# FengDushuo/BBBP-Multi-Modal-Deep-Ensemble-Framework

Measured on AMD Instinct MI355X. Metric: molecules/sec fwd+bwd (3-branch ensemble, B=512), higher is better.
Workload: dtype f32; 1 GPU; MixedInputModel F=167 (MACCS) + 3x128x128 image, 6-layer encoder + 2-stage CNN + fusion + BN head; forward + MSE + backward + fused AdamW, train mode (dropout 0.1); global_batch=512, per_gpu_batch=512, parallelism=dp1, input=device-resident

## Files before the change

bbbp-multi-modal-deep-ensemble-framework_amd/_lib.py:

```python
from __future__ import annotations

import ctypes
import os
import re
from ctypes import (POINTER, Structure, c_char_p, c_double, c_float, c_int, c_long, c_size_t, c_uint8, c_uint64, c_void_p)

_HERE = os.path.dirname(os.path.abspath(__file__))
LIB_PATH = os.environ.get("BBBP_LIB", os.path.join(_HERE, "libbbbp_hip.so"))
HEADER_PATH = os.path.join(os.path.dirname(_HERE), "include", "bbbp_hip.h")

_lib = None


class MixedDesc(Structure):
    _fields_ = [("batch", c_int), ("fingerprint_size", c_int), ("nhead", c_int), ("num_layers", c_int),
                ("dim_feedforward", c_int), ("training", c_int), ("dropout_p", c_float), ("seed", c_uint64),
                ("need_input_grad", c_int), ("fusion", c_int), ("inference", c_int),
                ("world", c_int), ("rank", c_int), ("collective", c_void_p), ("collective_ctx", c_void_p)]


CollectiveFn = ctypes.CFUNCTYPE(c_int, c_void_p, c_int, c_int, c_int, ctypes.c_size_t, ctypes.c_size_t, ctypes.c_size_t, c_void_p)


class GemmDesc(Structure):
# ... 91 lines not shown
    "bbbp_mlp_profile": (c_int, [c_int, c_void_p]),
    "bbbp_mlp_profile_groups": (c_int, [c_void_p, c_int]),
    "bbbp_set_conv_wgrad_beside_encoder": (c_int, [c_int]),
    "bbbp_set_conv2_fwd_pipe": (c_int, [c_int]),
    "bbbp_adamw_step_deferred": (c_int, [c_void_p, c_void_p, c_void_p, c_void_p, c_void_p, c_long, c_long, c_long, c_double, c_double, c_double, c_double, c_double, c_int, c_double]),
    "bbbp_param_sync": (c_int, [c_void_p]),
    "bbbp_param_stream": (c_void_p, []),
    "bbbp_scale": (c_int, [c_void_p, _FP, c_long, c_float]),
    "bbbp_resize_bilinear_totensor": (c_int, [c_void_p, c_void_p, c_void_p, c_void_p, _FP, c_void_p, c_void_p, c_int, c_void_p,
                                              c_void_p, c_int, c_int, c_int, c_int, c_int, c_int]),
    "bbbp_standardize_chunk": (c_int, [c_void_p, c_void_p, _FP, _FP, _FP, c_void_p, c_void_p, c_int, c_int, c_int]),
    "bbbp_set_partition": (c_int, [c_int, c_size_t]),
    "bbbp_set_comm_cus": (c_int, [c_int]),
    "bbbp_set_ln_absorb": (c_int, [c_int]),
    "bbbp_set_overlap": (c_int, [c_int]),
    "bbbp_profile_enable": (c_int, [c_int]),
    "bbbp_profile_select": (c_int, [ctypes.c_uint]),
    "bbbp_profile_num_sections": (c_int, []),
    "bbbp_profile_section_name": (c_char_p, [c_int]),
    "bbbp_profile_collect": (c_int, [POINTER(c_float), POINTER(c_int)]),
    "bbbp_profile_timeline": (c_int, [POINTER(c_int), POINTER(c_float), POINTER(c_float), c_int]),
    "bbbp_mixed_num_params": (c_int, [POINTER(MixedDesc)]),
    "bbbp_mixed_workspace_bytes": (c_size_t, [POINTER(MixedDesc)]),
    "bbbp_mixed_forward": (c_int, [c_void_p, POINTER(MixedDesc), _PP, _PP, _FP, _FP, _FP, c_void_p, c_size_t]),
    "bbbp_mixed_backward": (c_int, [c_void_p, POINTER(MixedDesc), _PP, _PP, _FP, _FP, _FP, c_void_p, c_size_t]),
}


def declared_symbols():
    text = open(HEADER_PATH).read()
    text = re.sub(r"/\*.*?\*/", "", text, flags=re.S)
    return sorted(set(re.findall(r"\b(bbbp_[a-z0-9_]+)\s*\(", text)))


def lib() -> ctypes.CDLL:
    global _lib
    if _lib is not None:
        return _lib
    if not os.path.exists(LIB_PATH):
        raise RuntimeError(
            f"{LIB_PATH} is missing: build it with `python -c 'import __graft_entry__ as g; g.build()'` "
            "(hipcc --offload-arch=gfx950).  The BBBP hot path has no CPU fallback.")
    l = ctypes.CDLL(LIB_PATH)
    for name, (res, args) in _SIGNATURES.items():
        fn = getattr(l, name)
        fn.restype = res
# ... 15 lines not shown
```

bbbp-multi-modal-deep-ensemble-framework_amd/csrc/engine.hip:

```cpp
#include "common.h"
#include "attention_b3.h"
#include "encoder_sliced.h"
#include "head_sync.h"
#include <optional>
#include "bbbp_hip.h"
#include <mutex>
#include <stdlib.h>

namespace {

constexpr int IMG = 128, C1 = 32, C2 = 64, FC = 128, NHEADS_FUSION = 4, FUS_HID = 128;
constexpr int H1 = 256, H2 = 128, H3 = 64;
constexpr int COMB = 2 * FC;
constexpr int IMG_FLAT = C2 * (IMG / 4) * (IMG / 4);

enum { L_INW = 0, L_INB, L_OUTW, L_OUTB, L_W1, L_B1, L_W2, L_B2, L_N1W, L_N1B, L_N2W, L_N2B, L_COUNT };
struct PIdx {
    int L, NF;
    PIdx(int layers, int fusion) : L(layers), NF(fusion == 0 ? 4 * NHEADS_FUSION : 0) {}
    explicit PIdx(const bbbp_mixed_desc* d) : PIdx(d->num_layers, d->fusion) {}
    int layer(int l, int k) const { return l * L_COUNT + k; }
    int base() const { return L * L_COUNT; }
    int fpfc_w() const { return base() + 0; }
    int fpfc_b() const { return base() + 1; }
// ... 110 lines not shown
        o.z1 = b.f(B * F); o.y1 = b.f(B * F); o.hff = b.f(B * DFF); o.z2 = b.f(B * F); o.y2 = b.f(B * F);
        o.mean1 = b.f(B); o.rstd1 = b.f(B); o.mean2 = b.f(B); o.rstd2 = b.f(B);
    }
    if (p->L > 0 && bbbp_enc_sliced_supported(p->B, p->F, p->NH, p->DFF, p->L)) {
        p->sl_sync = b.take(bbbp_enc_sliced_sync_bytes());
        p->sl_part = b.take(bbbp_enc_sliced_part_bytes(p->B, p->F));
        p->sl_kvpart = p->inference ? 0 : b.take(bbbp_enc_sliced_kvpart_bytes(p->B, p->F));
    } else {
        p->sl_sync = p->sl_part = p->sl_kvpart = 0;
    }
    for (int l = 0; l < p->L; ++l) {
        p->fwf[l] = p->fold ? b.f(bbbp_outproj_fold_floats(p->F, 0)) : 0; p->fbf[l] = p->fold ? b.f(bbbp_outproj_fold_floats(p->F, 1)) : 0;
        p->fwvt[l] = p->fold ? b.f(bbbp_outproj_fold_floats(p->F, 2)) : 0;
        p->ftdw[l] = (p->fold && !p->inference) ? b.f(bbbp_outproj_fold_floats(p->F, 3)) : 0;
        p->ftdb[l] = (p->fold && !p->inference) ? b.f(bbbp_outproj_fold_floats(p->F, 4)) : 0;
    }
    p->attn_part_bytes = p->attn_b3 ? bbbp_attn_b3_workspace_bytes(p->B, p->NH, p->D) : 0;
    p->attn_part = p->attn_part_bytes ? b.take(p->attn_part_bytes) : 0;
    p->pool1 = b.f(B * C1 * (IMG / 2) * (IMG / 2)); p->mask1 = p->inference ? 0 : b.take(B * C1 * (IMG / 2) * (IMG / 2));
    p->pool2 = b.f(B * IMG_FLAT); p->mask2 = p->inference ? 0 : b.take(B * IMG_FLAT);
    p->combined = b.f(B * COMB); p->hid = b.f(NHEADS_FUSION * B * FUS_HID); p->attn = b.f(B * NHEADS_FUSION);
    p->fused = p->concat ? p->combined : b.f(B * COMB); p->h = b.f(B * H1); p->hb = b.f(B * H1); p->bn_mean = b.f(H1); p->bn_rstd = b.f(H1);
    p->h2 = b.f(B * H2); p->h3 = b.f(B * H3);
    p->head_partial = b.f((size_t)p->world * ((B + 15) / 16) * 2 * H1);
    size_t cw = bbbp_conv3x3_workspace_bytes(p->B, 32, 64, 64, 64);
    size_t cw1 = bbbp_conv3x3_workspace_bytes(p->B, 3, 32, 128, 128);
    size_t sb = cw > cw1 ? cw : cw1;
    size_t gw = bbbp_gemm_workspace_bytes(p->B, FC, IMG_FLAT, 1);
    if (gw > sb) sb = gw;
    if (sb < ((size_t)32 << 20)) sb = (size_t)32 << 20;
    p->scratch_bytes = sb;
    p->scratch = b.take(sb);
    p->scratch2_bytes = (size_t)32 << 20;
    p->scratch2 = b.take(p->scratch2_bytes);
    if (p->inference) { p->total = b.off; return BBBP_OK; }
    for (int l = 0; l < p->L; ++l) {
        LayerGrad& g = p->lgrad[l];
        g.dyout = b.f(B * F); g.dz2 = b.f(B * F); g.dz2d = p->drop ? b.f(B * F) : g.dz2; g.dhff = b.f(B * DFF);
        g.dy1 = b.f(B * F); g.dz1 = b.f(B * F); g.dz1d = p->drop ? b.f(B * F) : g.dz1; g.dqkv = b.f(B * 3 * F);
    }
    p->scratch3_bytes = (size_t)32 << 20;
    p->scratch3 = b.take(p->scratch3_bytes);
    p->dA = b.f(B * F); p->dB = b.f(B * F); p->dqkv = b.f(B * 3 * F); p->dprob = p->flash ? 0 : b.f(NH * B * Bg); p->dctx = b.f(B * F);
    p->dkvg = p->exact ? b.f(Bg * 2 * F) : 0; p->dkvl = p->exact ? b.f(B * 2 * F) : 0;
    p->dhff = b.f(B * DFF); p->dpool2 = b.f(B * IMG_FLAT); p->dpool1 = b.f(B * C1 * (IMG / 2) * (IMG / 2));
    p->dcomb = b.f(B * COMB); p->dfused = b.f(B * COMB); p->dlogit = b.f(NHEADS_FUSION * B);
    p->dpre = b.f(NHEADS_FUSION * B * FUS_HID); p->dh = b.f(B * H1); p->dhb = b.f(B * H1); p->dh2 = b.f(B * H2);
// ... 304 lines not shown
        ms_sum[g_prof.sec[i]] += ms;
        count[g_prof.sec[i]] += 1;
    }
    g_prof.n = 0;
    return BBBP_OK;
}

extern "C" int bbbp_profile_timeline(int* section, float* start_ms, float* end_ms, int max_entries) {
    BBBP_CHECK_ARG(section && start_ms && end_ms && max_entries >= 0, "profile_timeline: bad arguments");
    const int n = g_prof.n < max_entries ? g_prof.n : max_entries;
    for (int i = 0; i < n; ++i) {
        section[i] = g_prof.sec[i];
        BBBP_CHECK_HIP(hipEventElapsedTime(&start_ms[i], g_prof.a[0], g_prof.a[i]));
        BBBP_CHECK_HIP(hipEventElapsedTime(&end_ms[i], g_prof.a[0], g_prof.b[i]));
    }
    return n;
}

extern "C" int bbbp_mixed_num_params(const bbbp_mixed_desc* d) {
    if (!d) return -1;
    if (d->num_layers < 0 || d->num_layers > 32 || (d->fusion != 0 && d->fusion != 1)) return -1;
    return PIdx(d).count();
}

extern "C" size_t bbbp_mixed_workspace_bytes(const bbbp_mixed_desc* d) {
    Plan p;
    if (make_plan(d, &p)) return 0;
    return p.total;
}

static int forward_enqueue(void* stream, const bbbp_mixed_desc* d, const float* const* P, float* const* bn_running,
                           const float* fingerprint, const float* image, float* out, void* workspace,
                           size_t workspace_bytes) {
    Plan plan;
    TRY(make_plan(d, &plan));
    SeedScope seed_scope(reinterpret_cast<const unsigned long long*>(static_cast<char*>(workspace) + plan.seed_slot));
    BBBP_CHECK_ARG(P && fingerprint && image && out && workspace && bn_running, "mixed_forward: null pointer");
    if (workspace_bytes < plan.total) {
        bbbp_set_error("mixed_forward: workspace %zu < %zu bytes", workspace_bytes, plan.total);
        return BBBP_ERR_WORKSPACE;
    }
    Ctx c{static_cast<hipStream_t>(stream), static_cast<char*>(workspace), &plan};
    const PIdx ix(d);
    if (bbbp_param_pending_elsewhere(P[ix.ifc_w()])) (void)bbbp_param_wait(c.st, nullptr);
    const int B = plan.B, F = plan.F, NH = plan.NH, D = plan.D, DFF = plan.DFF;
    const int Bk = (int)plan.Bg;
// ... 212 lines not shown
    if (!fused_rows && !sliced) {
        if (pend.z) {
            TRY(bbbp_layernorm_linear_fwd(ce.st, pend.z, F, pend.gamma, pend.beta, 1e-5f, P[ix.fpfc_w()], P[ix.fpfc_b()], comb, COMB, BBBP_ACT_RELU, 0.f, 0,
                                          pend.y, F, pend.mean, pend.rstd, B, FC, F));
            pend.z = nullptr;
        } else {
            TRY(linear_fwd(ce, x, F, P[ix.fpfc_w()], P[ix.fpfc_b()], comb, COMB, B, FC, F, BBBP_ACT_RELU));
        }
    }
    sec_enc.reset();

    if (ss) TRY(join_side(c.st, ss));
    part.reset();
    Section sec_head(c.st, SEC_HEAD_FWD);

    static const int fused_head = [] { const char* e = getenv("BBBP_FUSED_HEAD"); return e ? atoi(e) : 1; }();
    BBBP_CHECK_ARG(!plan.exact || (fused_head && NHEADS_FUSION == 4), "the exact-global-batch mode needs the fused head (BBBP_FUSED_HEAD=1)");
    if (fused_head && NHEADS_FUSION == 4) {
        const float *fw1[4] = {}, *fb1[4] = {}, *fw2[4] = {}, *fb2[4] = {};
        if (!plan.concat)
            for (int h = 0; h < 4; ++h) { fw1[h] = P[ix.fus(h, 0)]; fb1[h] = P[ix.fus(h, 1)]; fw2[h] = P[ix.fus(h, 2)]; fb2[h] = P[ix.fus(h, 3)]; }
        bbbp_head_sync sync;
        sync.world = plan.world; sync.rank = plan.rank;
        const size_t pcount = (size_t)((B + 15) / 16) * 2 * H1;
        if (plan.exact)
            sync.between = [&]() -> int {
                return run_collective(d, BBBP_COLL_ALLGATHER, BBBP_COLL_BN_FWD, -1, plan.head_partial + (size_t)plan.rank * pcount * sizeof(float),
                                      plan.head_partial, pcount, c.st);
            };
        return bbbp_head_forward_fused_sync(c.st, comb, fw1, fb1, fw2, fb2, P[ix.fc0_w()], P[ix.fc0_b()], P[ix.bn_w()], P[ix.bn_b()],
                                            bn_running[0], bn_running[1], P[ix.fc3_w()], P[ix.fc3_b()], P[ix.fc5_w()], P[ix.fc5_b()],
                                            P[ix.fc7_w()], P[ix.fc7_b()], c.f(plan.hid), c.f(plan.attn), c.f(plan.fused), c.f(plan.h),
                                            c.f(plan.hb), c.f(plan.bn_mean), c.f(plan.bn_rstd), c.f(plan.h2), c.f(plan.h3), out,
                                            c.f(plan.head_partial), B, d->training, plan.concat ? 1 : 0, plan.exact ? &sync : nullptr);
    }
    float* hid = c.f(plan.hid);
    float* fused = c.f(plan.fused);
    if (!plan.concat) {
        const float* w2[NHEADS_FUSION]; const float* b2[NHEADS_FUSION];
        for (int h = 0; h < NHEADS_FUSION; ++h) {
            TRY(linear_fwd(c, comb, COMB, P[ix.fus(h, 0)], P[ix.fus(h, 1)], hid + (size_t)h * B * FUS_HID, FUS_HID, B, FUS_HID, COMB,
                           BBBP_ACT_TANH));
            w2[h] = P[ix.fus(h, 2)]; b2[h] = P[ix.fus(h, 3)];
        }
        TRY(bbbp_fusion_combine_fwd(c.st, comb, hid, w2, b2, fused, c.f(plan.attn), B, COMB, FUS_HID, NHEADS_FUSION));
    }

// ... 63 lines not shown
    float* dlogit = c.f(plan.dlogit); float* dpre = c.f(plan.dpre);
    bool head_leaves_pending = false;
    auto head_leaves = [&]() -> int {
        TRY(linear_bwd_weight_bias(cl, dout, 1, h3, H3, G[ix.fc7_w()], G[ix.fc7_b()], B, 1, H3));
        TRY(linear_bwd_weight_bias(cl, dh3, H3, h2, H2, G[ix.fc5_w()], G[ix.fc5_b()], B, H3, H2));
        TRY(linear_bwd_weight_bias(cl, dh2, H2, hb, H1, G[ix.fc3_w()], G[ix.fc3_b()], B, H2, H1));
        TRY(linear_bwd_weight_bias(cl, dh, H1, fused, COMB, G[ix.fc0_w()], G[ix.fc0_b()], B, H1, COMB));
        for (int hh = 0; hh < (plan.concat ? 0 : NHEADS_FUSION); ++hh) {
            float* dl = dlogit + (size_t)hh * B;
            float* dp = dpre + (size_t)hh * B * FUS_HID;
            const float* hd = hid + (size_t)hh * B * FUS_HID;
            TRY(linear_bwd_weight_bias(cl, dl, 1, hd, FUS_HID, G[ix.fus(hh, 2)], G[ix.fus(hh, 3)], B, 1, FUS_HID));
            TRY(linear_bwd_weight_bias(cl, dp, FUS_HID, comb, COMB, G[ix.fus(hh, 0)], G[ix.fus(hh, 1)], B, FUS_HID, COMB));
        }
        TRY(bbbp_bias_act_bwd(cl.st, dcomb + FC, COMB, nullptr, 0, G[ix.ifc_b()], B, FC, 0, 1.f));
        return BBBP_OK;
    };
    BBBP_CHECK_ARG(!plan.exact || fused_head_bwd, "the exact-global-batch mode needs the fused head backward (bbbp_set_fused_head_bwd(1))");
    if (fused_head_bwd) {
        const float* fw1[NHEADS_FUSION]; const float* fw2[NHEADS_FUSION];
        for (int hh = 0; hh < NHEADS_FUSION; ++hh) { fw1[hh] = P[ix.fus(hh, 0)]; fw2[hh] = P[ix.fus(hh, 2)]; }
        bbbp_head_sync sync;
        sync.world = plan.world; sync.rank = plan.rank;
        const size_t pcount = (size_t)((B + 15) / 16) * 2 * H1;
        if (plan.exact)
            sync.between = [&]() -> int {
                return run_collective(d, BBBP_COLL_ALLGATHER, BBBP_COLL_BN_BWD, -1, plan.head_partial + (size_t)plan.rank * pcount * sizeof(float),
                                      plan.head_partial, pcount, c.st);
            };
        TRY(bbbp_head_backward_fused_sync(c.st, dout, comb, hid, c.f(plan.attn), h, h2, h3, c.f(plan.bn_mean), c.f(plan.bn_rstd),
                                          P[ix.bn_w()], fw1, fw2, P[ix.fc0_w()], P[ix.fc3_w()], P[ix.fc5_w()], P[ix.fc7_w()], dh3, dh2, dhb,
                                          dh, dlogit, dpre, dcomb, G[ix.bn_w()], G[ix.bn_b()], c.f(plan.head_partial), B, d->training,
                                          plan.exact ? &sync : nullptr));
        TRY(leaf_after(c));
        head_leaves_pending = true;
    } else {
    TRY(linear_bwd_weight_bias(cl, dout, 1, h3, H3, G[ix.fc7_w()], G[ix.fc7_b()], B, 1, H3));
    {
        bbbp_gemm_desc g = gemm_desc(0, 0, B, H3, 1, 1.f, dout, 1, P[ix.fc7_w()], H3, dh3, H3);
        g.gate = h3; g.ldg = H3;
        TRY(bbbp_gemm_f32_grouped(c.st, &g, 1, c.scratch(), c.scratch_bytes()));
    }
    TRY(leaf_after(c));
    TRY(linear_bwd_weight_bias(cl, dh3, H3, h2, H2, G[ix.fc5_w()], G[ix.fc5_b()], B, H3, H2));
    {
        bbbp_gemm_desc g = gemm_desc(0, 0, B, H2, H3, 1.f, dh3, H3, P[ix.fc5_w()], H2, dh2, H2);
        g.gate = h2; g.ldg = H2;
// ... 470 lines not shown
```

bbbp-multi-modal-deep-ensemble-framework_amd/csrc/head.hip:

```cpp
#include "common.h"
#include "bbbp_hip.h"
#include "head_sync.h"

namespace {

constexpr int ROWS = 16;
constexpr int NTH = 512;
constexpr int NW = NTH / 64;
constexpr int COMB = 256, FHID = 128, NHEADS = 4, H1 = 256, H2 = 128, H3 = 64;
constexpr int LD = COMB + 4;
typedef float f32x4g __attribute__((ext_vector_type(4), aligned(4)));
static_assert(NTH >= H1, "one thread per BatchNorm column");

struct HeadParams {
    const float* comb;
    const float* fw1[NHEADS]; const float* fb1[NHEADS]; const float* fw2[NHEADS]; const float* fb2[NHEADS];
    const float* w0; const float* b0;
    const float* gamma; const float* beta; float* running_mean; float* running_var;
    const float* w3; const float* b3;
    const float* w5; const float* b5;
    const float* w7; const float* b7;
    float* hid; float* attn; float* fused; float* h; float* hb; float* bn_mean; float* bn_rstd; float* h2; float* h3; float* out;
    float* partial;
    int B, training;
    float eps, momentum;
    int concat;
    int world, rank;
};

template <int NCH>
__device__ __forceinline__ void load_b(f32x4 (&bf)[NCH], const float* Wrow ) {
#pragma unroll
    for (int c = 0; c < NCH; ++c) { f32x4g v = *reinterpret_cast<const f32x4g*>(Wrow + 16 * c); bf[c] = f32x4{v[0], v[1], v[2], v[3]}; }
}
template <int NCH>
__device__ __forceinline__ f32x4 mma_tile(const f32x4 (&af)[NCH], const f32x4 (&bf)[NCH]) {
    f32x4 acc0 = {0.f, 0.f, 0.f, 0.f}, acc1 = {0.f, 0.f, 0.f, 0.f};
#pragma unroll
    for (int c = 0; c < NCH; ++c)
#pragma unroll
        for (int j = 0; j < 4; j += 2) {
            acc0 = __builtin_amdgcn_mfma_f32_16x16x4f32(af[c][j], bf[c][j], acc0, 0, 0, 0);
            acc1 = __builtin_amdgcn_mfma_f32_16x16x4f32(af[c][j + 1], bf[c][j + 1], acc1, 0, 0, 0);
        }
    return acc0 + acc1;
}

template <int NCH>
__device__ __forceinline__ void load_a(f32x4 (&af)[NCH], const float* s, int ld, int lane) {
    const int i = lane & 15, kq = lane >> 4;
#pragma unroll
    for (int c = 0; c < NCH; ++c) af[c] = *reinterpret_cast<const f32x4*>(s + i * ld + 16 * c + 4 * kq);
}

__device__ __forceinline__ float sum16(float v) {
    v += __shfl_xor(v, 1); v += __shfl_xor(v, 2); v += __shfl_xor(v, 4); v += __shfl_xor(v, 8);
    return v;
}

__global__ __launch_bounds__(NTH) void head_a_kernel(HeadParams p) {
    __shared__ __attribute__((aligned(16))) float sC[ROWS * LD];
    __shared__ float sLogit[NW][NHEADS][ROWS];
    __shared__ float sP[ROWS][NHEADS];
    const int t = threadIdx.x, lane = t & 63, wave = t >> 6;
    const int q = lane & 15, kq = lane >> 4;
    const int r0 = blockIdx.x * ROWS, nrows = min(ROWS, p.B - r0);
    for (int idx = t; idx < ROWS * (COMB / 4); idx += NTH) {
        const int r = idx / (COMB / 4), c4 = idx % (COMB / 4);
        f32x4 v = {0.f, 0.f, 0.f, 0.f};
        if (r < nrows) v = *reinterpret_cast<const f32x4*>(p.comb + (long)(r0 + r) * COMB + c4 * 4);
        *reinterpret_cast<f32x4*>(sC + r * LD + c4 * 4) = v;
    }
    __syncthreads();
    f32x4 af[COMB / 16];
    load_a<COMB / 16>(af, sC, LD, lane);
    float lg[NHEADS][4];
    f32x4 bf[2][COMB / 16];
    const int n = wave * 16 + q;
    if (p.concat) {
        load_b<COMB / 16>(bf[0], p.w0 + (long)n * COMB + 4 * kq);
    } else {
    load_b<COMB / 16>(bf[0], p.fw1[0] + (long)n * COMB + 4 * kq);
#pragma unroll
    for (int h = 0; h < NHEADS; ++h) {
        if (h + 1 < NHEADS) load_b<COMB / 16>(bf[(h + 1) & 1], p.fw1[h + 1] + (long)n * COMB + 4 * kq);
        else load_b<COMB / 16>(bf[(h + 1) & 1], p.w0 + (long)n * COMB + 4 * kq);
        f32x4 acc = mma_tile<COMB / 16>(af, bf[h & 1]);
        const float b = p.fb1[h][n], w2 = p.fw2[h][n];
#pragma unroll
        for (int r = 0; r < 4; ++r) {
            const int row = 4 * kq + r;
            const float v = tanhf(acc[r] + b);
            if (row < nrows) p.hid[((long)h * p.B + r0 + row) * FHID + n] = v;
            lg[h][r] = sum16(v * w2);
        }
    }
    if (q == 0) {
#pragma unroll
        for (int h = 0; h < NHEADS; ++h)
#pragma unroll
            for (int r = 0; r < 4; ++r) sLogit[wave][h][4 * kq + r] = lg[h][r];
    }
    __syncthreads();
    if (t < ROWS) {
        float a[NHEADS], m = -INFINITY;
#pragma unroll
        for (int h = 0; h < NHEADS; ++h) {
            float z = 0.f;
#pragma unroll
            for (int w = 0; w < NW; ++w) z += sLogit[w][h][t];
            a[h] = z + p.fb2[h][0];
            m = fmaxf(m, a[h]);
        }
        float den = 0.f;
#pragma unroll
        for (int h = 0; h < NHEADS; ++h) { a[h] = __expf(a[h] - m); den += a[h]; }
#pragma unroll
        for (int h = 0; h < NHEADS; ++h) {
            a[h] /= den;
            sP[t][h] = a[h];
            if (t < nrows) p.attn[(long)(r0 + t) * NHEADS + h] = a[h];
        }
    }
    __syncthreads();
    for (int idx = t; idx < ROWS * COMB; idx += NTH) {
        const int r = idx / COMB, c = idx % COMB;
        const float x = sC[r * LD + c];
        float s = 0.f;
#pragma unroll
        for (int h = 0; h < NHEADS; ++h) s += sP[r][h] * x;
        sC[r * LD + c] = s;
        if (r < nrows) p.fused[(long)(r0 + r) * COMB + c] = s;
    }
    __syncthreads();
    load_a<COMB / 16>(af, sC, LD, lane);
    }
#pragma unroll
    for (int tt = 0; tt < 2; ++tt) {
        const int n0 = (wave + NW * tt) * 16 + q;
        if (tt == 0) load_b<COMB / 16>(bf[1], p.w0 + (long)((wave + NW) * 16 + q) * COMB + 4 * kq);
        f32x4 acc = mma_tile<COMB / 16>(af, bf[tt & 1]);
        const float b = p.b0[n0];
        float v[4], s = 0.f;
#pragma unroll
        for (int r = 0; r < 4; ++r) {
            const int row = 4 * kq + r;
            v[r] = fmaxf(acc[r] + b, 0.f);
            if (row < nrows) { p.h[(long)(r0 + row) * H1 + n0] = v[r]; s += v[r]; }
        }
        s += __shfl_xor(s, 16); s += __shfl_xor(s, 32);
        const float mean = s / nrows;
        float m2 = 0.f;
#pragma unroll
        for (int r = 0; r < 4; ++r) if (4 * kq + r < nrows) { const float d = v[r] - mean; m2 += d * d; }
        m2 += __shfl_xor(m2, 16); m2 += __shfl_xor(m2, 32);
        if (kq == 0) {
            const long slot = (long)p.rank * gridDim.x + blockIdx.x;
            p.partial[(slot * 2 + 0) * H1 + n0] = mean;
            p.partial[(slot * 2 + 1) * H1 + n0] = m2;
        }
    }
}

__global__ __launch_bounds__(NTH) void head_b_kernel(HeadParams p) {
    __shared__ __attribute__((aligned(16))) float sA[ROWS * LD];
    __shared__ __attribute__((aligned(16))) float sB[ROWS * (H2 + 4)];
    __shared__ __attribute__((aligned(16))) float sD[ROWS * (H3 + 4)];
    __shared__ float sMean[H1], sRstd[H1];
    const int t = threadIdx.x, lane = t & 63, wave = t >> 6;
    const int q = lane & 15, kq = lane >> 4;
    const int r0 = blockIdx.x * ROWS, nrows = min(ROWS, p.B - r0);
    const int nblocks = (p.B + ROWS - 1) / ROWS;
    f32x4 bf3[H1 / 16];
    load_b<H1 / 16>(bf3, p.w3 + (long)(wave * 16 + q) * H1 + 4 * kq);
    if (t < H1) {
        const int c = t;
        float mean, rstd;
        if (p.training) {
            float na = 0.f, ma = 0.f, m2a = 0.f;
            for (int b = 0; b < nblocks * p.world; ++b) {
                const float nb = (float)min(ROWS, p.B - (b % nblocks) * ROWS);
                const float mb = p.partial[((long)b * 2 + 0) * H1 + c], m2b = p.partial[((long)b * 2 + 1) * H1 + c];
                const float d = mb - ma, n = na + nb;
                ma += d * (nb / n);
                m2a += m2b + d * d * (na * nb / n);
                na = n;
            }
            const float nall = (float)p.B * (float)p.world;
            const float var = m2a / nall;
            mean = ma; rstd = rsqrtf(var + p.eps);
            if (blockIdx.x == 0) {
                p.running_mean[c] = (1.f - p.momentum) * p.running_mean[c] + p.momentum * mean;
                p.running_var[c] = (1.f - p.momentum) * p.running_var[c] + p.momentum * var * (nall / (nall - 1.f));
            }
        } else {
// ... 141 lines not shown
                    p.dhb[(long)(r0 + row) * H1 + n] = g;
                    pa += g * (p.h[(long)(r0 + row) * H1 + n] - mu) * rs;
                    pb += g;
                }
            }
            sPa[kq][n] = pa; sPb[kq][n] = pb;
        }
    }
    __syncthreads();
    if (t < H1) {
        const long slot = (long)p.rank * gridDim.x + blockIdx.x;
        p.partial[(slot * 2 + 0) * H1 + t] = ((sPa[0][t] + sPa[1][t]) + sPa[2][t]) + sPa[3][t];
        p.partial[(slot * 2 + 1) * H1 + t] = ((sPb[0][t] + sPb[1][t]) + sPb[2][t]) + sPb[3][t];
    }
}

__global__ __launch_bounds__(NTH) void head_bwd_c_kernel(HeadBwdParams p) {
    __shared__ __attribute__((aligned(16))) float sX[ROWS * LD];
    __shared__ __attribute__((aligned(16))) float sP[NHEADS * ROWS * LDP];
    __shared__ float sSa[H1], sSb[H1];
    const int t = threadIdx.x, lane = t & 63, wave = t >> 6;
    const int q = lane & 15, kq = lane >> 4;
    const int r0 = blockIdx.x * ROWS, nrows = min(ROWS, p.B - r0);
    const int nblocks = (p.B + ROWS - 1) / ROWS;
    if (t < H1) {
        float sa = 0.f, sb = 0.f, la = 0.f, lb = 0.f;
        for (int b = 0; b < nblocks * p.world; ++b) {
            const float va = p.partial[((long)b * 2 + 0) * H1 + t], vb = p.partial[((long)b * 2 + 1) * H1 + t];
            sa += va; sb += vb;
            if (b / nblocks == p.rank) { la += va; lb += vb; }
        }
        sSa[t] = sa; sSb[t] = sb;
        if (blockIdx.x == 0) { p.dgamma[t] = la; p.dbeta[t] = lb; }
    }
    __syncthreads();
    for (int idx = t; idx < ROWS * H1; idx += NTH) {
        const int r = idx / H1, c = idx % H1;
        float v = 0.f;
        if (r < nrows) {
            const float d = p.dhb[(long)(r0 + r) * H1 + c], xv = p.h[(long)(r0 + r) * H1 + c];
            const float g = p.gamma[c], mu = p.bn_mean[c], rs = p.bn_rstd[c];
            const float nall = (float)p.B * (float)p.world;
            v = p.training ? g * rs * (d - sSb[c] / nall - (xv - mu) * rs * (sSa[c] / nall)) : d * g * rs;
            v = xv > 0.f ? v : 0.f;
            p.dh[(long)(r0 + r) * H1 + c] = v;
        }
        sX[r * LD + c] = v;
// ... 38 lines not shown
                sP[(hh * ROWS + r) * LDP + c] = v;
            }
        }
    }
    __syncthreads();
    f32x4 acc[2] = {{0.f, 0.f, 0.f, 0.f}, {0.f, 0.f, 0.f, 0.f}};
#pragma unroll
    for (int hh = 0; hh < NHEADS; ++hh) mma_kmajor<FHID, 2>(acc, sP + hh * ROWS * LDP, LDP, p.fw1[hh], COMB, wave * 32, lane);
#pragma unroll
    for (int u = 0; u < 2; ++u) {
        const int n = wave * 32 + 2 * q + u;
#pragma unroll
        for (int r = 0; r < 4; ++r) {
            const int row = 4 * kq + r;
            if (row < nrows) {
                const float v = acc[u][r] + sX[row * LD + n];
                p.dcomb[(long)(r0 + row) * COMB + n] = p.comb[(long)(r0 + row) * COMB + n] > 0.f ? v : 0.f;
            }
        }
    }
}

}

int bbbp_head_forward_fused(hipStream_t st, const float* comb, const float* const* fw1, const float* const* fb1,
                            const float* const* fw2, const float* const* fb2, const float* w0, const float* b0, const float* gamma,
                            const float* beta, float* running_mean, float* running_var, const float* w3, const float* b3,
                            const float* w5, const float* b5, const float* w7, const float* b7, float* hid, float* attn, float* fused,
                            float* h, float* hb, float* bn_mean, float* bn_rstd, float* h2, float* h3, float* out, float* partial,
                            int B, int training, int concat) {
    return bbbp_head_forward_fused_sync(st, comb, fw1, fb1, fw2, fb2, w0, b0, gamma, beta, running_mean, running_var, w3, b3, w5, b5, w7, b7,
                                        hid, attn, fused, h, hb, bn_mean, bn_rstd, h2, h3, out, partial, B, training, concat, nullptr);
}

int bbbp_head_forward_fused_sync(hipStream_t st, const float* comb, const float* const* fw1, const float* const* fb1,
                                 const float* const* fw2, const float* const* fb2, const float* w0, const float* b0, const float* gamma,
                                 const float* beta, float* running_mean, float* running_var, const float* w3, const float* b3,
                                 const float* w5, const float* b5, const float* w7, const float* b7, float* hid, float* attn, float* fused,
                                 float* h, float* hb, float* bn_mean, float* bn_rstd, float* h2, float* h3, float* out, float* partial,
                                 int B, int training, int concat, const bbbp_head_sync* sync) {
    const int world = sync ? sync->world : 1, rank = sync ? sync->rank : 0;
    BBBP_CHECK_ARG(B >= 1, "head: empty batch");
    BBBP_CHECK_ARG(world >= 1 && rank >= 0 && rank < world, "head: rank %d of %d", rank, world);
    BBBP_CHECK_ARG(!(training && (long)B * world <= 1), "Expected more than 1 value per channel when training, got input size [%d, %d]", B, H1);
    HeadParams p;
    p.comb = comb;
    for (int i = 0; i < NHEADS; ++i) { p.fw1[i] = fw1[i]; p.fb1[i] = fb1[i]; p.fw2[i] = fw2[i]; p.fb2[i] = fb2[i]; }
    p.w0 = w0; p.b0 = b0; p.gamma = gamma; p.beta = beta; p.running_mean = running_mean; p.running_var = running_var;
    p.w3 = w3; p.b3 = b3; p.w5 = w5; p.b5 = b5; p.w7 = w7; p.b7 = b7;
    p.hid = hid; p.attn = attn; p.fused = fused; p.h = h; p.hb = hb; p.bn_mean = bn_mean; p.bn_rstd = bn_rstd; p.h2 = h2; p.h3 = h3;
    p.out = out; p.partial = partial; p.B = B; p.training = training; p.eps = 1e-5f; p.momentum = 0.1f; p.concat = concat;
    p.world = world; p.rank = rank;
    const int blocks = cdiv(B, ROWS);
    hipLaunchKernelGGL(head_a_kernel, dim3(blocks), dim3(NTH), 0, st, p);
    BBBP_CHECK_LAUNCH();
    if (sync && sync->between && training) { const int rc = sync->between(); if (rc) return rc; }
    hipLaunchKernelGGL(head_b_kernel, dim3(blocks), dim3(NTH), 0, st, p);
    BBBP_CHECK_LAUNCH();
    return BBBP_OK;
}

int bbbp_head_backward_fused(hipStream_t st, const float* dout, const float* comb, const float* hid, const float* attn, const float* h,
                             const float* h2, const float* h3, const float* bn_mean, const float* bn_rstd, const float* gamma,
                             const float* const* fw1, const float* const* fw2, const float* w0, const float* w3, const float* w5,
                             const float* w7, float* dh3, float* dh2, float* dhb, float* dh, float* dlogit, float* dpre, float* dcomb,
                             float* dgamma, float* dbeta, float* partial, int B, int training) {
    return bbbp_head_backward_fused_sync(st, dout, comb, hid, attn, h, h2, h3, bn_mean, bn_rstd, gamma, fw1, fw2, w0, w3, w5, w7, dh3, dh2, dhb, dh,
                                         dlogit, dpre, dcomb, dgamma, dbeta, partial, B, training, nullptr);
}

int bbbp_head_backward_fused_sync(hipStream_t st, const float* dout, const float* comb, const float* hid, const float* attn, const float* h,
                                  const float* h2, const float* h3, const float* bn_mean, const float* bn_rstd, const float* gamma,
                                  const float* const* fw1, const float* const* fw2, const float* w0, const float* w3, const float* w5,
                                  const float* w7, float* dh3, float* dh2, float* dhb, float* dh, float* dlogit, float* dpre, float* dcomb,
                                  float* dgamma, float* dbeta, float* partial, int B, int training, const bbbp_head_sync* sync) {
    const int world = sync ? sync->world : 1, rank = sync ? sync->rank : 0;
    BBBP_CHECK_ARG(world >= 1 && rank >= 0 && rank < world, "head backward: rank %d of %d", rank, world);
    BBBP_CHECK_ARG(B >= 1, "head backward: empty batch");
    HeadBwdParams p;
    p.dout = dout; p.comb = comb; p.hid = hid; p.attn = attn; p.h = h; p.h2 = h2; p.h3 = h3;
    p.bn_mean = bn_mean; p.bn_rstd = bn_rstd; p.gamma = gamma;
    for (int i = 0; i < NHEADS; ++i) { p.fw1[i] = fw1[i]; p.fw2[i] = fw2[i]; }
    p.w0 = w0; p.w3 = w3; p.w5 = w5; p.w7 = w7;
    p.dh3 = dh3; p.dh2 = dh2; p.dhb = dhb; p.dh = dh; p.dlogit = dlogit; p.dpre = dpre; p.dcomb = dcomb;
    p.dgamma = dgamma; p.dbeta = dbeta; p.partial = partial; p.B = B; p.training = training;
    p.world = world; p.rank = rank;
    const int blocks = cdiv(B, ROWS);
    hipLaunchKernelGGL(head_bwd_a_kernel, dim3(blocks), dim3(NTH), 0, st, p);
    BBBP_CHECK_LAUNCH();
    if (sync && sync->between && training) { const int rc = sync->between(); if (rc) return rc; }
    hipLaunchKernelGGL(head_bwd_c_kernel, dim3(blocks), dim3(NTH), 0, st, p);
    BBBP_CHECK_LAUNCH();
    return BBBP_OK;
}
```

bbbp-multi-modal-deep-ensemble-framework_amd/csrc/head_sync.h:

```cpp
#pragma once
#include <functional>
#include <hip/hip_runtime.h>

struct bbbp_head_sync {
    int world = 1, rank = 0;
    std::function<int()> between;
};

int bbbp_head_forward_fused_sync(hipStream_t st, const float* comb, const float* const* fw1, const float* const* fb1,
                                 const float* const* fw2, const float* const* fb2, const float* w0, const float* b0, const float* gamma,
                                 const float* beta, float* running_mean, float* running_var, const float* w3, const float* b3,
                                 const float* w5, const float* b5, const float* w7, const float* b7, float* hid, float* attn, float* fused,
                                 float* h, float* hb, float* bn_mean, float* bn_rstd, float* h2, float* h3, float* out, float* partial,
                                 int B, int training, int concat, const bbbp_head_sync* sync);
int bbbp_head_backward_fused_sync(hipStream_t st, const float* dout, const float* comb, const float* hid, const float* attn, const float* h,
                                  const float* h2, const float* h3, const float* bn_mean, const float* bn_rstd, const float* gamma,
                                  const float* const* fw1, const float* const* fw2, const float* w0, const float* w3, const float* w5,
                                  const float* w7, float* dh3, float* dh2, float* dhb, float* dh, float* dlogit, float* dpre, float* dcomb,
                                  float* dgamma, float* dbeta, float* partial, int B, int training, const bbbp_head_sync* sync);
```

include/bbbp_hip.h:

```cpp
#ifndef BBBP_HIP_H
#define BBBP_HIP_H

#include <stddef.h>
#include <stdint.h>

#ifdef __cplusplus
extern "C" {
#endif

#define BBBP_OK 0
#define BBBP_ERR_ARG 1
#define BBBP_ERR_HIP 2
#define BBBP_ERR_WORKSPACE 3

#define BBBP_ACT_NONE 0
#define BBBP_ACT_RELU 1
#define BBBP_ACT_TANH 2

int bbbp_abi_version(void);
const char* bbbp_last_error(void);

size_t bbbp_gemm_workspace_bytes(int M, int N, int K, int batch);
int bbbp_gemm_f32(void* stream, int transA, int transB, int M, int N, int K, float alpha,
                  const float* A, int lda, const float* B, int ldb, float* C, int ldc,
// ... 109 lines not shown
enum { BBBP_COLL_KV = 0, BBBP_COLL_DKV = 1, BBBP_COLL_BN_FWD = 2, BBBP_COLL_BN_BWD = 3 };
typedef int (*bbbp_collective_fn)(void* ctx, int op, int what, int layer, size_t send_off, size_t recv_off, size_t count, void* stream);

typedef struct {
    int batch;
    int fingerprint_size;
    int nhead;
    int num_layers;
    int dim_feedforward;
    int training;
    float dropout_p;
    uint64_t seed;
    int need_input_grad;
    int fusion;
    int inference;
    int world;
    int rank;
    bbbp_collective_fn collective;
    void* collective_ctx;
} bbbp_mixed_desc;

int bbbp_mixed_num_params(const bbbp_mixed_desc* d);
size_t bbbp_mixed_workspace_bytes(const bbbp_mixed_desc* d);
int bbbp_mixed_forward(void* stream, const bbbp_mixed_desc* d, const float* const* params, float* const* bn_running,
                       const float* fingerprint, const float* image, float* out, void* workspace, size_t workspace_bytes);
int bbbp_mixed_backward(void* stream, const bbbp_mixed_desc* d, const float* const* params, float* const* grads,
                        const float* fingerprint, const float* image, const float* dout, void* workspace,
                        size_t workspace_bytes);

typedef struct bbbp_mlp_model {
    int n_layers;
    int units[5];
    int activation;
    int batch_size;
    int n_train;
    int n_iter_no_change, max_iter;
    double lr_init, alpha, beta1, beta2, eps, tol;
    double* params; double* adam_m; double* adam_v; double* grads;
    double* act; double* delta;
    const int* order;
    double* loss_curve;
    long t;
    double best_loss;
    int no_improve, n_iter, done;
} bbbp_mlp_model;
int bbbp_mlp_train_epochs(void* stream, bbbp_mlp_model* models_dev, int n_models, const double* X, const double* y,
// ... 51 lines not shown
```

Before: 216,100 molecules/s.

## Split fusion head forward kernel into per-head and per-column-group launches

Replaces the single head_a kernel, which ran one 512-thread block per 16 rows and looped over all four fusion heads plus two output tiles serially, with two kernels. The first runs one block per (row tile, fusion head) and writes logits to workspace. The second runs one block per (row tile, column group), recomputing the softmax and weighted fusion redundantly in each block before its own slice of the first head GEMM. This raises the block count at B=512 from 32 to 128 per launch to fill more CUs, at the cost of an extra launch, a logits round trip through global memory, and repeated row loads and softmax work.

```diff
diff --git a/bbbp-multi-modal-deep-ensemble-framework_amd/_lib.py b/bbbp-multi-modal-deep-ensemble-framework_amd/_lib.py
--- a/bbbp-multi-modal-deep-ensemble-framework_amd/_lib.py
+++ b/bbbp-multi-modal-deep-ensemble-framework_amd/_lib.py
@@ -137,6 +137,9 @@
     "bbbp_profile_timeline": (c_int, [POINTER(c_int), POINTER(c_float), POINTER(c_float), c_int]),
     "bbbp_mixed_num_params": (c_int, [POINTER(MixedDesc)]),
     "bbbp_mixed_workspace_bytes": (c_size_t, [POINTER(MixedDesc)]),
+    "bbbp_head_num_blocks": (c_int, [c_int]),
+    "bbbp_head_allgather_floats": (c_size_t, [c_int]),
+    "bbbp_head_workspace_floats": (c_size_t, [c_int, c_int]),
     "bbbp_mixed_forward": (c_int, [c_void_p, POINTER(MixedDesc), _PP, _PP, _FP, _FP, _FP, c_void_p, c_size_t]),
     "bbbp_mixed_backward": (c_int, [c_void_p, POINTER(MixedDesc), _PP, _PP, _FP, _FP, _FP, c_void_p, c_size_t]),
 }
diff --git a/bbbp-multi-modal-deep-ensemble-framework_amd/csrc/engine.hip b/bbbp-multi-modal-deep-ensemble-framework_amd/csrc/engine.hip
--- a/bbbp-multi-modal-deep-ensemble-framework_amd/csrc/engine.hip
+++ b/bbbp-multi-modal-deep-ensemble-framework_amd/csrc/engine.hip
@@ -156,7 +156,7 @@
     p->combined = b.f(B * COMB); p->hid = b.f(NHEADS_FUSION * B * FUS_HID); p->attn = b.f(B * NHEADS_FUSION);
     p->fused = p->concat ? p->combined : b.f(B * COMB); p->h = b.f(B * H1); p->hb = b.f(B * H1); p->bn_mean = b.f(H1); p->bn_rstd = b.f(H1);
     p->h2 = b.f(B * H2); p->h3 = b.f(B * H3);
-    p->head_partial = b.f((size_t)p->world * ((B + 15) / 16) * 2 * H1);
+    p->head_partial = b.f(bbbp_head_partial_floats(p->B, p->world));
     size_t cw = bbbp_conv3x3_workspace_bytes(p->B, 32, 64, 64, 64);
     size_t cw1 = bbbp_conv3x3_workspace_bytes(p->B, 3, 32, 128, 128);
     size_t sb = cw > cw1 ? cw : cw1;
@@ -507,6 +507,9 @@
     if (d->num_layers < 0 || d->num_layers > 32 || (d->fusion != 0 && d->fusion != 1)) return -1;
     return PIdx(d).count();
 }
+
+extern "C" size_t bbbp_head_allgather_floats(int B) { return B < 1 ? 0 : bbbp_head_slot_floats(B); }
+extern "C" size_t bbbp_head_workspace_floats(int B, int world) { return (B < 1 || world < 1) ? 0 : bbbp_head_partial_floats(B, world); }
 
 extern "C" size_t bbbp_mixed_workspace_bytes(const bbbp_mixed_desc* d) {
     Plan p;
@@ -765,7 +768,7 @@
             for (int h = 0; h < 4; ++h) { fw1[h] = P[ix.fus(h, 0)]; fb1[h] = P[ix.fus(h, 1)]; fw2[h] = P[ix.fus(h, 2)]; fb2[h] = P[ix.fus(h, 3)]; }
         bbbp_head_sync sync;
         sync.world = plan.world; sync.rank = plan.rank;
-        const size_t pcount = (size_t)((B + 15) / 16) * 2 * H1;
+        const size_t pcount = bbbp_head_slot_floats(B);
         if (plan.exact)
             sync.between = [&]() -> int {
                 return run_collective(d, BBBP_COLL_ALLGATHER, BBBP_COLL_BN_FWD, -1, plan.head_partial + (size_t)plan.rank * pcount * sizeof(float),
@@ -875,7 +878,7 @@
         for (int hh = 0; hh < NHEADS_FUSION; ++hh) { fw1[hh] = P[ix.fus(hh, 0)]; fw2[hh] = P[ix.fus(hh, 2)]; }
         bbbp_head_sync sync;
         sync.world = plan.world; sync.rank = plan.rank;
-        const size_t pcount = (size_t)((B + 15) / 16) * 2 * H1;
+        const size_t pcount = bbbp_head_slot_floats(B);
         if (plan.exact)
             sync.between = [&]() -> int {
                 return run_collective(d, BBBP_COLL_ALLGATHER, BBBP_COLL_BN_BWD, -1, plan.head_partial + (size_t)plan.rank * pcount * sizeof(float),
diff --git a/bbbp-multi-modal-deep-ensemble-framework_amd/csrc/head.hip b/bbbp-multi-modal-deep-ensemble-framework_amd/csrc/head.hip
--- a/bbbp-multi-modal-deep-ensemble-framework_amd/csrc/head.hip
+++ b/bbbp-multi-modal-deep-ensemble-framework_amd/csrc/head.hip
@@ -4,13 +4,17 @@
 
 namespace {
 
-constexpr int ROWS = 16;
+constexpr int ROWS = BBBP_HEAD_ROWS;
 constexpr int NTH = 512;
 constexpr int NW = NTH / 64;
 constexpr int COMB = 256, FHID = 128, NHEADS = 4, H1 = 256, H2 = 128, H3 = 64;
 constexpr int LD = COMB + 4;
 typedef float f32x4g __attribute__((ext_vector_type(4), aligned(4)));
+constexpr int CGROUPS = 4;
+constexpr int NTH2 = 64 * (H1 / 16 / CGROUPS);
 static_assert(NTH >= H1, "one thread per BatchNorm column");
+static_assert(ROWS == 16 && H1 == BBBP_HEAD_COLS && NHEADS == BBBP_HEAD_FUSION_HEADS, "head_sync.h describes these kernels");
+static_assert(FHID == 16 * NW, "head_a1: one hidden-layer tile per wave");
 
 struct HeadParams {
     const float* comb;
@@ -22,6 +26,7 @@
     const float* w7; const float* b7;
     float* hid; float* attn; float* fused; float* h; float* hb; float* bn_mean; float* bn_rstd; float* h2; float* h3; float* out;
     float* partial;
+    float* logit;
     int B, training;
     float eps, momentum;
     int concat;
@@ -58,107 +63,116 @@
     return v;
 }
 
-__global__ __launch_bounds__(NTH) void head_a_kernel(HeadParams p) {
+template <int NT>
+__device__ __forceinline__ void load_rows(float* sC, const float* comb, int r0, int nrows, int t) {
+    for (int idx = t; idx < ROWS * (COMB / 4); idx += NT) {
+        const int r = idx / (COMB / 4), c4 = idx % (COMB / 4);
+        f32x4 v = {0.f, 0.f, 0.f, 0.f};
+        if (r < nrows) v = *reinterpret_cast<const f32x4*>(comb + (long)(r0 + r) * COMB + c4 * 4);
+        *reinterpret_cast<f32x4*>(sC + r * LD + c4 * 4) = v;
+    }
+}
+
+__device__ __forceinline__ const float* pick(const float* const (&a)[NHEADS], int h) {
+    const float* r = a[0];
+#pragma unroll
+    for (int i = 1; i < NHEADS; ++i) r = h == i ? a[i] : r;
+    return r;
+}
+
+__global__ __launch_bounds__(NTH) void head_a1_kernel(HeadParams p) {
     __shared__ __attribute__((aligned(16))) float sC[ROWS * LD];
-    __shared__ float sLogit[NW][NHEADS][ROWS];
+    __shared__ float sLogit[NW][ROWS];
+    const int t = threadIdx.x, lane = t & 63, wave = t >> 6;
+    const int q = lane & 15, kq = lane >> 4;
+    const int r0 = blockIdx.x * ROWS, nrows = min(ROWS, p.B - r0);
+    const int h = blockIdx.y, n = wave * 16 + q;
+    f32x4 bf[COMB / 16];
+    load_b<COMB / 16>(bf, pick(p.fw1, h) + (long)n * COMB + 4 * kq);
+    const float b = pick(p.fb1, h)[n], w2 = pick(p.fw2, h)[n];
+    load_rows<NTH>(sC, p.comb, r0, nrows, t);
+    __syncthreads();
+    f32x4 af[COMB / 16];
+    load_a<COMB / 16>(af, sC, LD, lane);
+    const f32x4 acc = mma_tile<COMB / 16>(af, bf);
+#pragma unroll
+    for (int r = 0; r < 4; ++r) {
+        const int row = 4 * kq + r;
+        const float v = tanhf(acc[r] + b);
+        if (row < nrows) p.hid[((long)h * p.B + r0 + row) * FHID + n] = v;
+        const float lg = sum16(v * w2);
+        if (q == 0) sLogit[wave][row] = lg;
+    }
+    __syncthreads();
+    if (t < nrows) {
+        float z = 0.f;
+#pragma unroll
+        for (int w = 0; w < NW; ++w) z += sLogit[w][t];
+        p.logit[(long)(r0 + t) * NHEADS + h] = z + pick(p.fb2, h)[0];
+    }
+}
+
+__global__ __launch_bounds__(NTH2) void head_a2_kernel(HeadParams p) {
+    __shared__ __attribute__((aligned(16))) float sC[ROWS * LD];
     __shared__ float sP[ROWS][NHEADS];
     const int t = threadIdx.x, lane = t & 63, wave = t >> 6;
     const int q = lane & 15, kq = lane >> 4;
     const int r0 = blockIdx.x * ROWS, nrows = min(ROWS, p.B - r0);
-    for (int idx = t; idx < ROWS * (COMB / 4); idx += NTH) {
-        const int r = idx / (COMB / 4), c4 = idx % (COMB / 4);
-        f32x4 v = {0.f, 0.f, 0.f, 0.f};
-        if (r < nrows) v = *reinterpret_cast<const f32x4*>(p.comb + (long)(r0 + r) * COMB + c4 * 4);
-        *reinterpret_cast<f32x4*>(sC + r * LD + c4 * 4) = v;
+    const int cg = blockIdx.y, n0 = (cg * (NTH2 / 64) + wave) * 16 + q;
+    f32x4 bf[COMB / 16];
+    load_b<COMB / 16>(bf, p.w0 + (long)n0 * COMB + 4 * kq);
+    load_rows<NTH2>(sC, p.comb, r0, nrows, t);
+    if (!p.concat) {
+        if (t < ROWS) {
+            float a[NHEADS], m = -INFINITY;
+#pragma unroll
+            for (int h = 0; h < NHEADS; ++h) {
+                a[h] = t < nrows ? p.logit[(long)(r0 + t) * NHEADS + h] : 0.f;
+                m = fmaxf(m, a[h]);
+            }
+            float den = 0.f;
+#pragma unroll
+            for (int h = 0; h < NHEADS; ++h) { a[h] = __expf(a[h] - m); den += a[h]; }
+#pragma unroll
+            for (int h = 0; h < NHEADS; ++h) {
+                a[h] /= den;
+                sP[t][h] = a[h];
+                if (cg == 0 && t < nrows) p.attn[(long)(r0 + t) * NHEADS + h] = a[h];
+            }
+        }
+        __syncthreads();
+        for (int idx = t; idx < ROWS * COMB; idx += NTH2) {
+            const int r = idx / COMB, c = idx % COMB;
+            const float x = sC[r * LD + c];
+            float s = 0.f;
+#pragma unroll
+            for (int h = 0; h < NHEADS; ++h) s += sP[r][h] * x;
+            sC[r * LD + c] = s;
+            if (r < nrows && c / (COMB / CGROUPS) == cg) p.fused[(long)(r0 + r) * COMB + c] = s;
+        }
     }
     __syncthreads();
     f32x4 af[COMB / 16];
     load_a<COMB / 16>(af, sC, LD, lane);
-    float lg[NHEADS][4];
-    f32x4 bf[2][COMB / 16];
-    const int n = wave * 16 + q;
-    if (p.concat) {
-        load_b<COMB / 16>(bf[0], p.w0 + (long)n * COMB + 4 * kq);
-    } else {
-    load_b<COMB / 16>(bf[0], p.fw1[0] + (long)n * COMB + 4 * kq);
-#pragma unroll
-    for (int h = 0; h < NHEADS; ++h) {
-        if (h + 1 < NHEADS) load_b<COMB / 16>(bf[(h + 1) & 1], p.fw1[h + 1] + (long)n * COMB + 4 * kq);
-        else load_b<COMB / 16>(bf[(h + 1) & 1], p.w0 + (long)n * COMB + 4 * kq);
-        f32x4 acc = mma_tile<COMB / 16>(af, bf[h & 1]);
-        const float b = p.fb1[h][n], w2 = p.fw2[h][n];
-#pragma unroll
-        for (int r = 0; r < 4; ++r) {
-            const int row = 4 * kq + r;
-            const float v = tanhf(acc[r] + b);
-            if (row < nrows) p.hid[((long)h * p.B + r0 + row) * FHID + n] = v;
-            lg[h][r] = sum16(v * w2);
-        }
-    }
-    if (q == 0) {
-#pragma unroll
-        for (int h = 0; h < NHEADS; ++h)
-#pragma unroll
-            for (int r = 0; r < 4; ++r) sLogit[wave][h][4 * kq + r] = lg[h][r];
-    }
-    __syncthreads();
-    if (t < ROWS) {
-        float a[NHEADS], m = -INFINITY;
-#pragma unroll
-        for (int h = 0; h < NHEADS; ++h) {
-            float z = 0.f;
-#pragma unroll
-            for (int w = 0; w < NW; ++w) z += sLogit[w][h][t];
-            a[h] = z + p.fb2[h][0];
-            m = fmaxf(m, a[h]);
-        }
-        float den = 0.f;
-#pragma unroll
-        for (int h = 0; h < NHEADS; ++h) { a[h] = __expf(a[h] - m); den += a[h]; }
-#pragma unroll
-        for (int h = 0; h < NHEADS; ++h) {
-            a[h] /= den;
-            sP[t][h] = a[h];
-            if (t < nrows) p.attn[(long)(r0 + t) * NHEADS + h] = a[h];
-        }
-    }
-    __syncthreads();
-    for (int idx = t; idx < ROWS * COMB; idx += NTH) {
-        const int r = idx / COMB, c = idx % COMB;
-        const float x = sC[r * LD + c];
-        float s = 0.f;
-#pragma unroll
-        for (int h = 0; h < NHEADS; ++h) s += sP[r][h] * x;
-        sC[r * LD + c] = s;
-        if (r < nrows) p.fused[(long)(r0 + r) * COMB + c] = s;
-    }
-    __syncthreads();
-    load_a<COMB / 16>(af, sC, LD, lane);
-    }
-#pragma unroll
-    for (int tt = 0; tt < 2; ++tt) {
-        const int n0 = (wave + NW * tt) * 16 + q;
-        if (tt == 0) load_b<COMB / 16>(bf[1], p.w0 + (long)((wave + NW) * 16 + q) * COMB + 4 * kq);
-        f32x4 acc = mma_tile<COMB / 16>(af, bf[tt & 1]);
-        const float b = p.b0[n0];
-        float v[4], s = 0.f;
-#pragma unroll
-        for (int r = 0; r < 4; ++r) {
-            const int row = 4 * kq + r;
-            v[r] = fmaxf(acc[r] + b, 0.f);
-            if (row < nrows) { p.h[(long)(r0 + row) * H1 + n0] = v[r]; s += v[r]; }
-        }
-        s += __shfl_xor(s, 16); s += __shfl_xor(s, 32);
-        const float mean = s / nrows;
-        float m2 = 0.f;
-#pragma unroll
-        for (int r = 0; r < 4; ++r) if (4 * kq + r < nrows) { const float d = v[r] - mean; m2 += d * d; }
-        m2 += __shfl_xor(m2, 16); m2 += __shfl_xor(m2, 32);
-        if (kq == 0) {
-            const long slot = (long)p.rank * gridDim.x + blockIdx.x;
-            p.partial[(slot * 2 + 0) * H1 + n0] = mean;
-            p.partial[(slot * 2 + 1) * H1 + n0] = m2;
-        }
+    const f32x4 acc = mma_tile<COMB / 16>(af, bf);
+    const float b = p.b0[n0];
+    float v[4], s = 0.f;
+#pragma unroll
+    for (int r = 0; r < 4; ++r) {
+        const int row = 4 * kq + r;
+        v[r] = fmaxf(acc[r] + b, 0.f);
+        if (row < nrows) { p.h[(long)(r0 + row) * H1 + n0] = v[r]; s += v[r]; }
+    }
+    s += __shfl_xor(s, 16); s += __shfl_xor(s, 32);
+    const float mean = s / nrows;
+    float m2 = 0.f;
+#pragma unroll
+    for (int r = 0; r < 4; ++r) if (4 * kq + r < nrows) { const float d = v[r] - mean; m2 += d * d; }
+    m2 += __shfl_xor(m2, 16); m2 += __shfl_xor(m2, 32);
+    if (kq == 0) {
+        const long slot = (long)p.rank * gridDim.x + blockIdx.x;
+        p.partial[(slot * 2 + 0) * H1 + n0] = mean;
+        p.partial[(slot * 2 + 1) * H1 + n0] = m2;
     }
 }
 
@@ -170,7 +184,7 @@
     const int t = threadIdx.x, lane = t & 63, wave = t >> 6;
     const int q = lane & 15, kq = lane >> 4;
     const int r0 = blockIdx.x * ROWS, nrows = min(ROWS, p.B - r0);
-    const int nblocks = (p.B + ROWS - 1) / ROWS;
+    const int nblocks = bbbp_head_blocks(p.B);
     f32x4 bf3[H1 / 16];
     load_b<H1 / 16>(bf3, p.w3 + (long)(wave * 16 + q) * H1 + 4 * kq);
     if (t < H1) {
@@ -358,7 +372,7 @@
     const int t = threadIdx.x, lane = t & 63, wave = t >> 6;
     const int q = lane & 15, kq = lane >> 4;
     const int r0 = blockIdx.x * ROWS, nrows = min(ROWS, p.B - r0);
-    const int nblocks = (p.B + ROWS - 1) / ROWS;
+    const int nblocks = bbbp_head_blocks(p.B);
     if (t < H1) {
         float sa = 0.f, sb = 0.f, la = 0.f, lb = 0.f;
         for (int b = 0; b < nblocks * p.world; ++b) {
@@ -443,6 +457,8 @@
 }
 
 }
+
+extern "C" int bbbp_head_num_blocks(int B) { return B < 1 ? 0 : bbbp_head_blocks(B); }
 
 int bbbp_head_forward_fused(hipStream_t st, const float* comb, const float* const* fw1, const float* const* fb1,
                             const float* const* fw2, const float* const* fb2, const float* w0, const float* b0, const float* gamma,
@@ -472,8 +488,13 @@
     p.hid = hid; p.attn = attn; p.fused = fused; p.h = h; p.hb = hb; p.bn_mean = bn_mean; p.bn_rstd = bn_rstd; p.h2 = h2; p.h3 = h3;
     p.out = out; p.partial = partial; p.B = B; p.training = training; p.eps = 1e-5f; p.momentum = 0.1f; p.concat = concat;
     p.world = world; p.rank = rank;
-    const int blocks = cdiv(B, ROWS);
-    hipLaunchKernelGGL(head_a_kernel, dim3(blocks), dim3(NTH), 0, st, p);
+    const int blocks = bbbp_head_blocks(B);
+    p.logit = partial + (size_t)world * bbbp_head_slot_floats(B);
+    if (!concat) {
+        hipLaunchKernelGGL(head_a1_kernel, dim3(blocks, NHEADS), dim3(NTH), 0, st, p);
+        BBBP_CHECK_LAUNCH();
+    }
+    hipLaunchKernelGGL(head_a2_kernel, dim3(blocks, CGROUPS), dim3(NTH2), 0, st, p);
     BBBP_CHECK_LAUNCH();
     if (sync && sync->between && training) { const int rc = sync->between(); if (rc) return rc; }
     hipLaunchKernelGGL(head_b_kernel, dim3(blocks), dim3(NTH), 0, st, p);
@@ -506,7 +527,7 @@
     p.dh3 = dh3; p.dh2 = dh2; p.dhb = dhb; p.dh = dh; p.dlogit = dlogit; p.dpre = dpre; p.dcomb = dcomb;
     p.dgamma = dgamma; p.dbeta = dbeta; p.partial = partial; p.B = B; p.training = training;
     p.world = world; p.rank = rank;
-    const int blocks = cdiv(B, ROWS);
+    const int blocks = bbbp_head_blocks(B);
     hipLaunchKernelGGL(head_bwd_a_kernel, dim3(blocks), dim3(NTH), 0, st, p);
     BBBP_CHECK_LAUNCH();
     if (sync && sync->between && training) { const int rc = sync->between(); if (rc) return rc; }
diff --git a/bbbp-multi-modal-deep-ensemble-framework_amd/csrc/head_sync.h b/bbbp-multi-modal-deep-ensemble-framework_amd/csrc/head_sync.h
--- a/bbbp-multi-modal-deep-ensemble-framework_amd/csrc/head_sync.h
+++ b/bbbp-multi-modal-deep-ensemble-framework_amd/csrc/head_sync.h
@@ -1,6 +1,17 @@
 #pragma once
+#include <cstddef>
 #include <functional>
 #include <hip/hip_runtime.h>
+
+constexpr int BBBP_HEAD_ROWS = 16;
+constexpr int BBBP_HEAD_COLS = 256;
+constexpr int BBBP_HEAD_FUSION_HEADS = 4;
+
+__host__ __device__ inline int bbbp_head_blocks(int B) { return (B + BBBP_HEAD_ROWS - 1) / BBBP_HEAD_ROWS; }
+__host__ __device__ inline size_t bbbp_head_slot_floats(int B) { return (size_t)bbbp_head_blocks(B) * 2 * BBBP_HEAD_COLS; }
+__host__ __device__ inline size_t bbbp_head_partial_floats(int B, int world) {
+    return (size_t)world * bbbp_head_slot_floats(B) + (size_t)B * BBBP_HEAD_FUSION_HEADS;
+}
 
 struct bbbp_head_sync {
     int world = 1, rank = 0;
diff --git a/include/bbbp_hip.h b/include/bbbp_hip.h
--- a/include/bbbp_hip.h
+++ b/include/bbbp_hip.h
@@ -155,6 +155,9 @@
 
 int bbbp_mixed_num_params(const bbbp_mixed_desc* d);
 size_t bbbp_mixed_workspace_bytes(const bbbp_mixed_desc* d);
+int bbbp_head_num_blocks(int B);
+size_t bbbp_head_allgather_floats(int B);
+size_t bbbp_head_workspace_floats(int B, int world);
 int bbbp_mixed_forward(void* stream, const bbbp_mixed_desc* d, const float* const* params, float* const* bn_running,
                        const float* fingerprint, const float* image, float* out, void* workspace, size_t workspace_bytes);
 int bbbp_mixed_backward(void* stream, const bbbp_mixed_desc* d, const float* const* params, float* const* grads,
```

Measured after the change: 217,400 molecules/s, median of 6. No clear change (+0.6%).
